# wengflow/robust-e-nerf

Measured on AMD Instinct MI355X. Metric: train_rays_per_sec, higher is better.
Workload: dtype f32; 1 GPU; BASELINE configs[1]: synthetic ficus-like event stream, 65536 events/step/GPU = 2 renders x 65536 rays x 128 samples, arch ngp, fp32, l_diff (2 renders), fwd+bwd+Adam; sampler=uniform; sampler=uniform, samples_per_ray=128, parallelism=dp1, front_prefetched=False, mlp_precision=highest, device_counts=False, device_count_overflows=0, fwd_chunks=8, dist_world_size=1

## Files before the change

robust_e_nerf_amd/csrc/ren_hashgrid_binned.hip:

```cpp
#include <cstdlib>
#include "ren_hashgrid_common.h"

namespace {

constexpr int BIN_SHIFT = 13;
constexpr int BIN_ENTRIES = 1 << BIN_SHIFT;
constexpr int MAX_BINS_PER_LEVEL = 64;
constexpr int MAX_BINS = REN_MAX_LEVELS * MAX_BINS_PER_LEVEL;
#ifndef REN_SC_THREADS
#define REN_SC_THREADS 512
#endif
#ifndef REN_SC_WAVES
#define REN_SC_WAVES 6
#endif
#ifndef REN_SC_WAVES_PAIR
#define REN_SC_WAVES_PAIR 8
#endif
constexpr int SC_THREADS = REN_SC_THREADS;
constexpr int SC_ENTRIES = SC_THREADS * 8;
constexpr int CNT_THREADS = 1024, CNT_SAMPLES = 1024;
constexpr int64_t PART_ENTRIES_MIN = 1 << 16, PART_ENTRIES_MAX = 1 << 23;
constexpr int N_SUB = 8;
__device__ __forceinline__ int xcd_id() {
    unsigned x;
    asm volatile("s_getreg_b32 %0, hwreg(HW_REG_XCC_ID)" : "=s"(x));
    return (int)(x & (N_SUB - 1));
}
inline int64_t part_entries_for(int64_t n, int64_t hashed_cap) {
    int64_t p = hashed_cap;
    if (p == 0) {
        p = PART_ENTRIES_MIN;
        while (p < (1 << 21) && p * 1024 < n * 128) p <<= 1;
    }
    return p < PART_ENTRIES_MIN ? PART_ENTRIES_MIN : (p > PART_ENTRIES_MAX ? PART_ENTRIES_MAX : p);
}
constexpr int LMAX_SLOTS = 8, LMAX_STRIDE = 32;
constexpr int LMAX_WORDS = REN_MAX_LEVELS * LMAX_SLOTS * LMAX_STRIDE;

struct BinTab {
    int bin_base[REN_MAX_LEVELS + 1];
    uint32_t cap[REN_MAX_LEVELS];
    uint32_t pair[REN_MAX_LEVELS];
    uint32_t skip[REN_MAX_LEVELS];
    int sub_by_xcd;
    int cnt_stride;
    int halve;
};

struct Part {
    uint32_t gbin, single;
    uint64_t begin, end;
};

struct Workspace {
    uint32_t *counts, *level_max, *cursors, *n_parts;
    uint32_t *bin_cap;
    uint64_t *bin_start;
    Part *parts;
    char *pool;
};
constexpr int PAIR_BIN_SHIFT = 26;

struct TanSrc {
    const float *rays_do, *rays_dd, *dfeatd;
};

__device__ __forceinline__ void lds_barrier() { asm volatile("s_waitcnt lgkmcnt(0)\n\ts_barrier" ::: "memory"); }

struct SampleArgs {
    int layout;
    const float *dfeat, *x_unit;
    ren_scene_dev sc;
    const float *rays_o, *rays_d;
    const int32_t *ray_indices;
    const float *t_starts, *t_ends;
    int64_t n;
    TanSrc tan;
    const int64_t *n_dev;
};

template <bool TAN>
__device__ __forceinline__ void unit_pos(const SampleArgs &a, int64_t i, float *u, float *ud) {
    ud[0] = 0.f; ud[1] = 0.f; ud[2] = 0.f;
    if (TAN) {
        float x[3], xd[3];
        sample_pos_jvp(a.rays_o, a.rays_d, a.tan.rays_do, a.tan.rays_dd, a.ray_indices, a.t_starts, a.t_ends, i, x, xd);
        contract_jvp(a.sc, x, xd, u, ud);
    } else if (a.x_unit) {
        u[0] = a.x_unit[3 * i]; u[1] = a.x_unit[3 * i + 1]; u[2] = a.x_unit[3 * i + 2];
    } else {
        float x, y, z; int ray;
        ren_sample_pos(a.rays_o, a.rays_d, a.ray_indices, a.t_starts, a.t_ends, i, x, y, z, ray);
        ren_contract(a.sc, x, y, z, u[0], u[1], u[2]);
    }
}

template <bool TAN>
__device__ __forceinline__ bool load_dfeat(const SampleArgs &a, int n_levels, int lvl, int64_t i, float &d0, float &d1,
                                           float &e0, float &e1) {
    e0 = 0.f; e1 = 0.f;
    if (TAN || a.layout == 1) {
        const int64_t b = ((i >> 5) * REN_MAX_LEVELS + lvl) * 64 + (i & 31);
        d0 = a.dfeat[b]; d1 = a.dfeat[b + 32];
        if (TAN) { e0 = a.tan.dfeatd[b]; e1 = a.tan.dfeatd[b + 32]; }
    } else {
        const float2 d = reinterpret_cast<const float2 *>(a.dfeat)[i * n_levels + lvl];
        d0 = d.x; d1 = d.y;
    }
    return d0 != 0.f || d1 != 0.f || e0 != 0.f || e1 != 0.f;
}


constexpr int RUN_LANES = 16;

template <int OFF>
__device__ __forceinline__ float dpp_shr(float v) {
    return __int_as_float(__builtin_amdgcn_update_dpp(0, __float_as_int(v), 0x110 | OFF, 0xf, 0xf, true));
}
template <int OFF>
__device__ __forceinline__ int dpp_shr_i(int v) { return __builtin_amdgcn_update_dpp(0, v, 0x110 | OFF, 0xf, 0xf, true); }

__device__ __forceinline__ bool run_tail(bool dense, bool have, uint32_t key, int lane, bool &head) {
    if (!dense) { head = true; return have; }
    const uint32_t k = have ? key : 0x80000000u | (uint32_t)lane;
    const uint32_t kp = __shfl_up(k, 1, 64), kn = __shfl_down(k, 1, 64);
    const int sub = lane & (RUN_LANES - 1);
    head = !(sub > 0 && have && kp == k);
    return have && (sub == RUN_LANES - 1 || kn != k);
}

template <int OFF>
__device__ __forceinline__ void run_merge_step(int &f, float (&v0)[8], float (&v1)[8]) {
    const float take = f ? 0.f : 1.f;
#pragma unroll
    for (int c = 0; c < 8; ++c) {
        v0[c] = fmaf(dpp_shr<OFF>(v0[c]), take, v0[c]);
        v1[c] = fmaf(dpp_shr<OFF>(v1[c]), take, v1[c]);
    }
    f |= dpp_shr_i<OFF>(f);
}

__device__ __forceinline__ void run_merge(bool head, int lane, float (&v0)[8], float (&v1)[8]) {
    int f = head ? 1 : 0;
    run_merge_step<1>(f, v0, v1);
    run_merge_step<2>(f, v0, v1);
    run_merge_step<4>(f, v0, v1);
    run_merge_step<8>(f, v0, v1);
}

__device__ __forceinline__ uint32_t bin_rank(bool dense, bool emit, uint32_t bin, int lane, uint32_t *hist) {
    if (!dense) return emit ? atomicAdd(&hist[bin], 1u) : 0u;
    uint32_t rank = 0;
    uint64_t todo = __ballot(emit);
    while (todo) {
        const int leader = __ffsll((unsigned long long)todo) - 1;
        const uint32_t b = __shfl(bin, leader, 64);
        const uint64_t m = __ballot(emit && bin == b);
        uint32_t base = 0;
        if (lane == leader) base = atomicAdd(&hist[b], (uint32_t)__popcll(m));
        base = __shfl(base, leader, 64);
        if (emit && bin == b) rank = base + (uint32_t)__popcll(m & ((1ull << lane) - 1ull));
        todo &= ~m;
    }
    return rank;
}

__device__ __forceinline__ void bin_rank8_dense(bool emit, const uint32_t (&bin)[8], int lane, uint32_t *hist, uint32_t (&rank)[8]) {
    const uint64_t m = __ballot(emit);
#pragma unroll
    for (int c = 0; c < 8; ++c) rank[c] = 0;
    if (!m) return;
    const int leader = __ffsll((unsigned long long)m) - 1;
    uint32_t lb[8];
    bool mixed = false;
#pragma unroll
    for (int c = 0; c < 8; ++c) {
        lb[c] = __shfl(bin[c], leader, 64);
        mixed |= emit && bin[c] != lb[c];
    }
    if (__ballot(mixed)) {
#pragma unroll
        for (int c = 0; c < 8; ++c) rank[c] = bin_rank(true, emit, bin[c], lane, hist);
        return;
    }
    const uint32_t cnt = (uint32_t)__popcll(m), pre = (uint32_t)__popcll(m & ((1ull << lane) - 1ull));
    uint32_t base[8] = {0, 0, 0, 0, 0, 0, 0, 0};
    if (lane == leader) {
#pragma unroll
        for (int c = 0; c < 8; ++c) base[c] = atomicAdd(&hist[lb[c]], cnt);
    }
#pragma unroll
    for (int c = 0; c < 8; ++c) rank[c] = __shfl(base[c], leader, 64) + pre;
}

template <bool TAN>
__global__ __launch_bounds__(CNT_THREADS) void bin_count_kernel(GridDev g, BinTab bt, SampleArgs a,
                                                                uint32_t *__restrict__ counts) {
    __shared__ uint32_t hist[MAX_BINS];
    for (int t = threadIdx.x; t < MAX_BINS; t += CNT_THREADS) hist[t] = 0;
    __syncthreads();
    const int lane = threadIdx.x & 63;
#pragma unroll 1
    for (int k = 0; k < CNT_SAMPLES / CNT_THREADS; ++k) {
        const int64_t i = (int64_t)blockIdx.x * bt.cnt_stride * CNT_SAMPLES + k * CNT_THREADS + threadIdx.x;
        const bool inb = i < ren_eff_n(a.n, a.n_dev);
        float u[3] = {0.f, 0.f, 0.f}, ud[3];
        if (inb) unit_pos<TAN>(a, i, u, ud);
#pragma unroll 1
        for (int lvl = 0; lvl < g.n_levels; ++lvl) {
            if (bt.cap[lvl] || bt.skip[lvl]) continue;
            float d0, d1, e0, e1;
            const bool have = inb && (a.dfeat == nullptr || load_dfeat<TAN>(a, g.n_levels, lvl, i, d0, d1, e0, e1));
            const LevelPos p = level_pos(u[0], u[1], u[2], g.scale[lvl]);
            const uint32_t res = g.res[lvl], size = g.size[lvl];
            const bool hashed = g.hashed[lvl] != 0;
            bool head;
            uint32_t idx[8];
            corner_indices8(p.c[0], p.c[1], p.c[2], res, size, hashed, idx);
            const bool emit = run_tail(!hashed, have, idx[0], lane, head);
#pragma unroll
            for (int c = 0; c < 8; ++c) (void)bin_rank(!hashed, emit, idx[c] >> BIN_SHIFT, lane, hist + lvl * MAX_BINS_PER_LEVEL);
        }
    }
    __syncthreads();
    for (int t = threadIdx.x; t < MAX_BINS; t += CNT_THREADS) {
        const int lvl = t / MAX_BINS_PER_LEVEL, bin = t % MAX_BINS_PER_LEVEL;
        if (lvl < g.n_levels && bin < bt.bin_base[lvl + 1] - bt.bin_base[lvl] && hist[t])
            atomicAdd(&counts[bt.bin_base[lvl] + bin], hist[t]);
    }
}

__global__ __launch_bounds__(MAX_BINS) void bin_offsets_kernel(int n_bins, BinTab bt, uint64_t capacity_slots,
                                                               const uint32_t *__restrict__ counts,
                                                               uint32_t *__restrict__ cursors,
                                                               uint32_t *__restrict__ bin_cap,
                                                               uint64_t *__restrict__ bin_start) {
    __shared__ uint64_t s_cnt[MAX_BINS];
    const int t = threadIdx.x;
    uint64_t c = 0, slots = 0;
    bool pair = false;
    if (t < n_bins) {
        int lvl = 0;
        while (lvl + 1 < REN_MAX_LEVELS && t >= bt.bin_base[lvl + 1]) ++lvl;
        pair = bt.pair[lvl] != 0;
        c = bt.skip[lvl] ? 0 : bt.cap[lvl] ? bt.cap[lvl] : counts[t];
        if (!bt.skip[lvl] && !bt.cap[lvl] && bt.cnt_stride > 1) c = c * bt.cnt_stride + c * bt.cnt_stride / 4 + 4096;
        if (bt.halve) c = c / 2;
        c &= ~(uint64_t)7;
        if (pair) c = (c / N_SUB) & ~(uint64_t)7;
        slots = pair ? c * N_SUB : (c * 10 + 15) / 16;
        for (int x = 0; x < N_SUB; ++x) cursors[t * N_SUB + x] = 0;
    }
    s_cnt[t] = slots;
    __syncthreads();
    for (int off = 1; off < MAX_BINS; off <<= 1) {
        const uint64_t a = t >= off ? s_cnt[t - off] : 0;
        __syncthreads();
        s_cnt[t] += a;
        __syncthreads();
    }
    if (t < n_bins) {
        const uint64_t start = s_cnt[t] - slots;
        uint64_t room = start < capacity_slots ? capacity_slots - start : 0;
        if (room > slots) room = slots;
        if (room < slots) c = (pair ? room / N_SUB : room * 16 / 10) & ~(uint64_t)7;
        bin_start[t] = start < capacity_slots ? start : capacity_slots;
        bin_cap[t] = (uint32_t)c;
    }
    if (t == n_bins - 1) bin_start[n_bins] = s_cnt[t] < capacity_slots ? s_cnt[t] : capacity_slots;
}

__global__ __launch_bounds__(MAX_BINS) void bin_partition_kernel(int n_bins, uint64_t PART_ENTRIES, BinTab bt,
                                                                 const uint32_t *__restrict__ cursors,
                                                                 const uint32_t *__restrict__ bin_cap,
                                                                 Part *__restrict__ parts, uint32_t *__restrict__ n_parts) {
    __shared__ uint32_t s_np[MAX_BINS];
    const int t = threadIdx.x;
    uint64_t c = 0;
    bool pair = false;
    if (t < n_bins) {
        int lvl = 0;
        while (lvl + 1 < REN_MAX_LEVELS && t >= bt.bin_base[lvl + 1]) ++lvl;
        pair = bt.pair[lvl] != 0;
        for (int x = 0; x < (pair ? N_SUB : 1); ++x) c += cursors[t * N_SUB + x] < bin_cap[t] ? cursors[t * N_SUB + x] : bin_cap[t];
    }
    const uint32_t np = pair ? (c ? 1u : 0u) : (uint32_t)((c + PART_ENTRIES - 1) / PART_ENTRIES);
    s_np[t] = np;
    __syncthreads();
    for (int off = 1; off < MAX_BINS; off <<= 1) {
        const uint32_t b = t >= off ? s_np[t - off] : 0;
        __syncthreads();
        s_np[t] += b;
        __syncthreads();
    }
    if (t == n_bins - 1) n_parts[0] = s_np[t];
    const uint32_t pbase = s_np[t] - np;
    for (uint32_t k = 0; k < np; ++k) {
        Part p;
        p.gbin = t; p.single = np == 1;
        p.begin = (uint64_t)k * PART_ENTRIES;
        p.end = k + 1 == np ? c : p.begin + PART_ENTRIES;
        parts[pbase + k] = p;
    }
}

__device__ __forceinline__ void table_atomic(float *grad_table, uint32_t offset, uint32_t idx, float a, float b) {
    float *gt = grad_table + 2 * ((size_t)offset + idx);
    atomicAdd(gt, a);
    atomicAdd(gt + 1, b);
}

template <bool TAN, int KIND>
__global__ __launch_bounds__(SC_THREADS, KIND == 1 ? REN_SC_WAVES_PAIR : REN_SC_WAVES) void bin_scatter_kernel(
    GridDev g, BinTab bt, SampleArgs a, Workspace ws, float *__restrict__ grad_table) {
    __shared__ uint32_t hist[MAX_BINS_PER_LEVEL], loc[MAX_BINS_PER_LEVEL + 1], fit[MAX_BINS_PER_LEVEL];
    __shared__ char *gp0[MAX_BINS_PER_LEVEL], *gp1[MAX_BINS_PER_LEVEL];
    __shared__ __attribute__((aligned(16))) unsigned char stage[KIND == 1 ? SC_THREADS * 4 * 16 : SC_ENTRIES * 12];
    __shared__ float wave_max[SC_THREADS / 64];
    __shared__ int any_overflow;
    uint32_t *st_key = reinterpret_cast<uint32_t *>(stage);
    float2 *st_v = reinterpret_cast<float2 *>(stage + SC_ENTRIES * 4);
    float4 *st_p = reinterpret_cast<float4 *>(stage);
    const int64_t chunk = blockIdx.x;
    const int tid = threadIdx.x, lane = tid & 63;
    const int64_t i = chunk * SC_THREADS + tid;
    const bool inb = i < ren_eff_n(a.n, a.n_dev);
    float u[3] = {0.f, 0.f, 0.f}, ud[3] = {0.f, 0.f, 0.f};
    if (inb) unit_pos<TAN>(a, i, u, ud);
    constexpr bool pairs = KIND == 1;
    const int sub = !pairs ? 0 : bt.sub_by_xcd ? xcd_id() : (int)((chunk >> 3) & (N_SUB - 1));
#pragma unroll 1
    for (int lvl = 0; lvl < g.n_levels; ++lvl) {
        if (bt.skip[lvl]) continue;
        if (KIND == 1 && !bt.pair[lvl]) continue;
        if (KIND == 2 && bt.pair[lvl]) continue;
        if (tid < MAX_BINS_PER_LEVEL) hist[tid] = 0;
        if (tid == 0) any_overflow = 0;
        lds_barrier();
        const uint32_t res = g.res[lvl], size = g.size[lvl];
        const bool hashed = g.hashed[lvl] != 0;
        const float scale = g.scale[lvl];
        float d0 = 0.f, d1 = 0.f, e0 = 0.f, e1 = 0.f;
        const bool valid = inb && load_dfeat<TAN>(a, g.n_levels, lvl, i, d0, d1, e0, e1);
        const LevelPos p = level_pos(u[0], u[1], u[2], scale);
        const float wx1 = p.w[0], wy1 = p.w[1], wz1 = p.w[2], wx0 = 1.f - wx1, wy0 = 1.f - wy1, wz0 = 1.f - wz1;
        if (!valid) { d0 = 0.f; d1 = 0.f; e0 = 0.f; e1 = 0.f; }
        uint32_t key[8];
        float v0[8], v1[8];
        bool have;
        float vmax = 0.f;
        uint32_t idx[8];
        corner_indices8(p.c[0], p.c[1], p.c[2], res, size, hashed, idx);
        if (pairs) {
            const bool same = ((idx[0] ^ idx[1]) >> BIN_SHIFT) == 0;
#pragma unroll
            for (int j = 0; j < 4; ++j) {
                const float wyz = ((j & 1) ? wy1 : wy0) * ((j & 2) ? wz1 : wz0);
                v0[j] = wyz * d0; v1[j] = wyz * d1;
            }
            if (valid && !same) {
#pragma unroll
                for (int j = 0; j < 4; ++j) {
                    table_atomic(grad_table, g.offset[lvl], idx[2 * j], wx0 * v0[j], wx0 * v1[j]);
                    table_atomic(grad_table, g.offset[lvl], idx[2 * j + 1], wx1 * v0[j], wx1 * v1[j]);
                }
            }
            have = valid && same;
#pragma unroll
            for (int j = 0; j < 4; ++j) {
                const uint32_t bin = idx[2 * j] >> BIN_SHIFT;
                key[4 + j] = have ? atomicAdd(&hist[bin], 1u) : 0u;
                key[j] = (idx[2 * j] & (BIN_ENTRIES - 1)) | ((idx[2 * j + 1] & (BIN_ENTRIES - 1)) << BIN_SHIFT) |
                         (bin << PAIR_BIN_SHIFT);
            }
            if (valid) vmax = fmaxf(fabsf(d0), fabsf(d1));
        } else {
            const float wxy[4] = {wx0 * wy0, wx1 * wy0, wx0 * wy1, wx1 * wy1};
#pragma unroll
            for (int c = 0; c < 8; ++c) {
                const float wz = (c & 4) ? wz1 : wz0;
                const float w = wxy[c & 3] * wz;
                v0[c] = w * d0; v1[c] = w * d1;
                if (TAN) {
                    const float wx = (c & 1) ? wx1 : wx0, wy = (c & 2) ? wy1 : wy0;
                    const float bx = (c & 1) ? ud[0] : -ud[0], by = (c & 2) ? ud[1] : -ud[1], bz = (c & 4) ? ud[2] : -ud[2];
                    const float wdc = scale * (bx * wy * wz + wx * by * wz + wxy[c & 3] * bz);
                    v0[c] += wdc * e0; v1[c] += wdc * e1;
                }
            }
            bool head;
            have = run_tail(!hashed, valid, idx[0], lane, head);
            if (!hashed) run_merge(head, lane, v0, v1);
            if (TAN) {
                if (have) {
#pragma unroll
                    for (int c = 0; c < 8; ++c) vmax = fmaxf(vmax, fmaxf(fabsf(v0[c]), fabsf(v1[c])));
                }
            } else if (valid) {
                vmax = fmaxf(fabsf(d0), fabsf(d1)) * (hashed ? 1.f : (float)RUN_LANES);
            }
            if (!hashed) {
                uint32_t bins[8], rk[8];
#pragma unroll
                for (int c = 0; c < 8; ++c) bins[c] = idx[c] >> BIN_SHIFT;
                bin_rank8_dense(have, bins, lane, hist, rk);
#pragma unroll
                for (int c = 0; c < 8; ++c) key[c] = (rk[c] << 19) | idx[c];
            } else {
#pragma unroll
                for (int c = 0; c < 8; ++c) {
                    const uint32_t rank = bin_rank(false, have, idx[c] >> BIN_SHIFT, lane, hist);
                    key[c] = (rank << 19) | idx[c];
                }
            }
        }
#pragma unroll
        for (int off = 32; off > 0; off >>= 1) vmax = fmaxf(vmax, __shfl_xor(vmax, off, 64));
        if (lane == 0) wave_max[tid >> 6] = vmax;
        lds_barrier();
        if (tid == SC_THREADS - 1) {
            float m = 0.f;
#pragma unroll
            for (int w = 0; w < SC_THREADS / 64; ++w) m = fmaxf(m, wave_max[w]);
            uint32_t *slot = ws.level_max + (lvl * LMAX_SLOTS + (int)(chunk % LMAX_SLOTS)) * LMAX_STRIDE;
            if (__float_as_uint(m) > __builtin_nontemporal_load(slot)) atomicMax(slot, __float_as_uint(m));
        }
        if (tid < MAX_BINS_PER_LEVEL) {
            const int nb = bt.bin_base[lvl + 1] - bt.bin_base[lvl];
            const uint32_t cnt = hist[tid];
            uint32_t inc = cnt;
#pragma unroll
            for (int off = 1; off < 64; off <<= 1) {
                const uint32_t t = __shfl_up(inc, off, 64);
                if (tid >= off) inc += t;
            }
            loc[tid] = inc - cnt;
            if (tid == MAX_BINS_PER_LEVEL - 1) loc[MAX_BINS_PER_LEVEL] = inc;
            uint32_t room = cnt;
            char *q0 = nullptr, *q1 = nullptr;
            if (tid < nb && cnt) {
                const int gb = bt.bin_base[lvl] + tid;
                const uint32_t at = atomicAdd(&ws.cursors[gb * N_SUB + sub], cnt);
                const uint32_t cap = ws.bin_cap[gb];
                room = at >= cap ? 0u : (cap - at < cnt ? cap - at : cnt);
                char *base = ws.pool + (ws.bin_start[gb] + (pairs ? (uint64_t)sub * cap : 0)) * 16;
                const int64_t first = (int64_t)at - (int64_t)(inc - cnt);
                if (pairs) q0 = base + first * 16;
                else { q0 = base + first * 8; q1 = base + (int64_t)cap * 8 + first * 2; }
            }
            fit[tid] = room;
            if (room < cnt) any_overflow = 1;
            gp0[tid] = q0; gp1[tid] = q1;
        }
        lds_barrier();
        if (have) {
            if (pairs) {
#pragma unroll
                for (int j = 0; j < 4; ++j)
                    st_p[loc[key[j] >> PAIR_BIN_SHIFT] + key[4 + j]] = make_float4(__uint_as_float(key[j]), v0[j], v1[j], wx1);
            } else {
#pragma unroll
                for (int c = 0; c < 8; ++c) {
                    const uint32_t ix = key[c] & 0x7FFFFu;
                    const uint32_t pos = loc[ix >> BIN_SHIFT] + (key[c] >> 19);
                    st_key[pos] = ix;
                    st_v[pos] = make_float2(v0[c], v1[c]);
                }
            }
        }
        lds_barrier();
        const uint32_t total = loc[MAX_BINS_PER_LEVEL];
        const bool ovf = any_overflow != 0;
        if (pairs) {
            for (uint32_t q = tid; q < total; q += SC_THREADS) {
                const float4 r = st_p[q];
                const uint32_t code = __float_as_uint(r.x), b = code >> PAIR_BIN_SHIFT;
                if (!ovf || q - loc[b] < fit[b]) {
                    reinterpret_cast<float4 *>(gp0[b])[q] = r;
                } else {
                    const uint32_t i0 = (b << BIN_SHIFT) | (code & (BIN_ENTRIES - 1));
                    const uint32_t i1 = (b << BIN_SHIFT) | ((code >> BIN_SHIFT) & (BIN_ENTRIES - 1));
                    table_atomic(grad_table, g.offset[lvl], i0, (1.f - r.w) * r.y, (1.f - r.w) * r.z);
                    table_atomic(grad_table, g.offset[lvl], i1, r.w * r.y, r.w * r.z);
                }
            }
            continue;
        }
        for (uint32_t q = tid; q < total; q += SC_THREADS) {
            const uint32_t ix = st_key[q], b = ix >> BIN_SHIFT;
            const float2 v = st_v[q];
            if (!ovf || q - loc[b] < fit[b]) {
                reinterpret_cast<uint16_t *>(gp1[b])[q] = (uint16_t)(ix & (BIN_ENTRIES - 1));
                reinterpret_cast<float2 *>(gp0[b])[q] = v;
            } else {
                table_atomic(grad_table, g.offset[lvl], ix, v.x, v.y);
            }
        }
    }
}

__device__ __forceinline__ long long to_fixed(float v, double scale) {
    return __double2ll_rn((double)v * scale);
}

__global__ __launch_bounds__(1024) void bin_accumulate_kernel(GridDev g, BinTab bt, Workspace ws,
                                                              float *__restrict__ grad_table) {
    extern __shared__ __attribute__((aligned(16))) unsigned long long acc[];
    if (blockIdx.x >= ws.n_parts[0]) return;
    const Part part = ws.parts[blockIdx.x];
    unsigned long long *acc0 = acc, *acc1 = acc + BIN_ENTRIES;
    for (int e = threadIdx.x; e < 2 * BIN_ENTRIES; e += 1024) acc[e] = 0ull;
    int lvl = 0;
    while (lvl + 1 < g.n_levels && (int)part.gbin >= bt.bin_base[lvl + 1]) ++lvl;
    int ex;
    uint32_t lmax = 0;
    for (int k = 0; k < LMAX_SLOTS; ++k) lmax = max(lmax, ws.level_max[(lvl * LMAX_SLOTS + k) * LMAX_STRIDE]);
    (void)frexpf(__uint_as_float(lmax), &ex);
    const double scale = ldexp(1.0, 38 - ex), inv_scale = ldexp(1.0, ex - 38);
    const char *base = ws.pool + ws.bin_start[part.gbin] * 16;
    const uint32_t first = ((uint32_t)part.gbin - bt.bin_base[lvl]) << BIN_SHIFT;
    const uint32_t lim = g.size[lvl] > first ? g.size[lvl] - first : 0;
    float2 *gt = reinterpret_cast<float2 *>(grad_table) + g.offset[lvl] + first;
    constexpr int FL = BIN_ENTRIES / 1024;
    float2 gv[FL];
#pragma unroll
    for (int u = 0; u < FL; ++u) {
        const uint32_t k = threadIdx.x + u * 1024;
        gv[u] = (part.single && k < lim) ? gt[k] : make_float2(0.f, 0.f);
    }
    __syncthreads();
    uint64_t e = part.begin + threadIdx.x;
    if (bt.pair[lvl]) {
        const float4 *rec = reinterpret_cast<const float4 *>(base);
        auto add = [&](const float4 &r) {
            const uint32_t code = __float_as_uint(r.x);
            const uint32_t i0 = code & (BIN_ENTRIES - 1), i1 = (code >> BIN_SHIFT) & (BIN_ENTRIES - 1);
            const float f0 = 1.f - r.w;
            atomicAdd(&acc0[i0], (unsigned long long)to_fixed(f0 * r.y, scale));
            atomicAdd(&acc1[i0], (unsigned long long)to_fixed(f0 * r.z, scale));
            atomicAdd(&acc0[i1], (unsigned long long)to_fixed(r.w * r.y, scale));
            atomicAdd(&acc1[i1], (unsigned long long)to_fixed(r.w * r.z, scale));
        };
        const uint32_t cap = ws.bin_cap[part.gbin];
        for (int x = 0; x < N_SUB; ++x) {
            const float4 *rx = rec + (size_t)x * cap;
            const uint32_t fill = ws.cursors[part.gbin * N_SUB + x];
            const uint64_t end = fill < cap ? fill : cap;
            uint64_t q = threadIdx.x;
            for (; q + 3 * 1024 < end; q += 4 * 1024) {
                float4 r[4];
#pragma unroll
                for (int u = 0; u < 4; ++u) r[u] = rx[q + u * 1024];
#pragma unroll
                for (int u = 0; u < 4; ++u) add(r[u]);
            }
            for (; q < end; q += 1024) add(rx[q]);
        }
    } else {
        const float2 *out_v = reinterpret_cast<const float2 *>(base);
        const uint16_t *out_idx = reinterpret_cast<const uint16_t *>(base + (size_t)ws.bin_cap[part.gbin] * 8);
        for (; e + 3 * 1024 < part.end; e += 4 * 1024) {
            uint32_t ix[4]; float2 v[4];
#pragma unroll
            for (int u = 0; u < 4; ++u) { ix[u] = out_idx[e + u * 1024]; v[u] = out_v[e + u * 1024]; }
#pragma unroll
            for (int u = 0; u < 4; ++u) {
                atomicAdd(&acc0[ix[u]], (unsigned long long)to_fixed(v[u].x, scale));
                atomicAdd(&acc1[ix[u]], (unsigned long long)to_fixed(v[u].y, scale));
            }
        }
        for (; e < part.end; e += 1024) {
            const uint32_t idx = out_idx[e];
            const float2 v = out_v[e];
            atomicAdd(&acc0[idx], (unsigned long long)to_fixed(v.x, scale));
            atomicAdd(&acc1[idx], (unsigned long long)to_fixed(v.y, scale));
        }
    }
    __syncthreads();
#pragma unroll
    for (int u = 0; u < FL; ++u) {
        const uint32_t k = threadIdx.x + u * 1024;
        if (k >= lim) continue;
        const long long qa = (long long)acc0[k], qb = (long long)acc1[k];
        if (qa == 0 && qb == 0) continue;
        const float a = (float)((double)qa * inv_scale), b = (float)((double)qb * inv_scale);
        if (part.single) {
            float2 v = gv[u];
            v.x += a; v.y += b;
            gt[k] = v;
        } else {
            atomicAdd(&gt[k].x, a);
            atomicAdd(&gt[k].y, b);
        }
    }
}

inline size_t align256(size_t v) { return (v + 255) & ~(size_t)255; }

struct Layout { size_t counts, level_max, cursors, n_parts, bin_cap, bin_start, parts, pool, total, slots; int64_t entries, max_parts; };

Layout make_layout(int64_t n) {
    Layout L;
    const size_t E = (size_t)n * 140 + (size_t)MAX_BINS * 4096 + 16 * 8 * 16 * CNT_SAMPLES;
    L.entries = (int64_t)E;
    L.slots = (E * 10 + 15) / 16 + MAX_BINS;
    L.max_parts = (int64_t)(E / PART_ENTRIES_MIN) + MAX_BINS + 1;
    size_t o = 0;
    L.counts = o; o += MAX_BINS * 4;
    L.level_max = o; o = align256(o + LMAX_WORDS * 4);
    L.cursors = o; o = align256(o + MAX_BINS * 4 * N_SUB);
    L.n_parts = o; o = align256(o + 4);
    L.bin_cap = o; o = align256(o + MAX_BINS * 4);
    L.bin_start = o; o = align256(o + (MAX_BINS + 1) * 8);
    L.parts = o; o = align256(o + (size_t)L.max_parts * sizeof(Part));
    L.pool = o; o = align256(o + L.slots * 16);
    L.total = o;
    return L;
}

}

extern "C" int64_t ren_hashgrid_bwd_binned_workspace_bytes(int64_t n) {
    if (n < 0) return -1;
    return (int64_t)make_layout(n).total;
}

static int binned_impl(const ren_grid_desc *grid, float *grad_table, const float *x_unit,
                       const ren_scene_desc *scene, const float *rays_o, const float *rays_d,
                       const int32_t *ray_indices, const float *t_starts, const float *t_ends,
                       int64_t n, int32_t layout, const float *dfeat, void *workspace,
                       void *stream, TanSrc tan, uint32_t level_mask = 0xFFFFFFFFu, int phases = 7,
                       int64_t first = 0, int64_t m = -1, const int64_t *n_dev = nullptr) {
    GridDev g;
    int rc = make_grid(grid, g);
    if (rc) return rc;
    const bool do_begin = phases & 1, do_scatter = phases & 2, do_finish = phases & 4;
    if (m < 0) m = n - first;
    if (!workspace || n < 0 || (layout != 0 && layout != 1) || first < 0 || m < 0 || first + m > n) return REN_ERR_BAD_ARG;
    if ((do_scatter && (!dfeat || !grad_table)) || (do_finish && !grad_table)) return REN_ERR_BAD_ARG;
    if (do_scatter && phases != 7 && ((first & 31) != 0 || tan.dfeatd)) return REN_ERR_BAD_ARG;
    const bool from_rays = x_unit == nullptr;
    if ((do_begin || do_scatter) && from_rays && (!scene || !rays_o || !rays_d || !ray_indices || !t_starts || !t_ends))
        return REN_ERR_BAD_ARG;
    if (layout == 1 && g.n_levels != REN_MAX_LEVELS) return REN_ERR_UNSUPPORTED;
    if (n >= ((int64_t)1 << 28)) return REN_ERR_UNSUPPORTED;
    BinTab bt;
    int nb = 0;
    for (int l = 0; l < REN_MAX_LEVELS; ++l) {
        bt.bin_base[l] = nb;
        if (l < g.n_levels) {
            if (g.size[l] > (uint32_t)(MAX_BINS_PER_LEVEL << BIN_SHIFT)) return REN_ERR_UNSUPPORTED;
            nb += (int)((g.size[l] + BIN_ENTRIES - 1) >> BIN_SHIFT);
        }
    }
    bt.bin_base[REN_MAX_LEVELS] = nb;
    for (int l = g.n_levels; l < REN_MAX_LEVELS; ++l) bt.bin_base[l] = nb;
    int64_t hashed_cap = 0;
    const bool use_pairs = !tan.dfeatd && ren_knob(REN_KNOB_HGB_NO_PAIRS) != 1;
    for (int l = 0; l < REN_MAX_LEVELS; ++l) {
        bt.cap[l] = 0;
        bt.pair[l] = 0;
        bt.skip[l] = l < g.n_levels && !((level_mask >> l) & 1u);
        if (l < g.n_levels && g.hashed[l]) {
            const int64_t bins = (g.size[l] + BIN_ENTRIES - 1) >> BIN_SHIFT;
            bt.pair[l] = use_pairs ? 1 : 0;
            const int64_t mean = ((use_pairs ? 4 : 8) * n + bins - 1) / bins;
            bt.cap[l] = use_pairs ? (uint32_t)(N_SUB * (((mean / N_SUB + mean / 400 + 1024) + 7) & ~(int64_t)7))
                                  : (uint32_t)(mean + mean / 50 + 4096);
            if ((int64_t)bt.cap[l] > hashed_cap) hashed_cap = bt.cap[l];
        }
    }
    const int64_t part_entries = part_entries_for(n, hashed_cap);
    if (n == 0) return REN_OK;
    ren_scene_dev sc = {};
    if (scene) sc = ren_make_scene(scene);
    const Layout L = make_layout(n);
    char *w = (char *)workspace;
    Workspace ws;
    ws.counts = (uint32_t *)(w + L.counts); ws.level_max = (uint32_t *)(w + L.level_max);
    ws.cursors = (uint32_t *)(w + L.cursors);
    ws.n_parts = (uint32_t *)(w + L.n_parts); ws.bin_cap = (uint32_t *)(w + L.bin_cap);
    ws.bin_start = (uint64_t *)(w + L.bin_start);
    ws.parts = (Part *)(w + L.parts); ws.pool = w + L.pool;
    hipStream_t st = (hipStream_t)stream;
    SampleArgs a;
    a.layout = layout; a.dfeat = dfeat; a.x_unit = x_unit; a.sc = sc; a.rays_o = rays_o; a.rays_d = rays_d;
    a.ray_indices = ray_indices; a.t_starts = t_starts; a.t_ends = t_ends; a.n = n; a.tan = tan;
    a.n_dev = n_dev;
    if (n_dev && phases != 7) return REN_ERR_BAD_ARG;
    bt.halve = ren_knob(REN_KNOB_HGB_HALVE_REGIONS) == 1;
    bt.sub_by_xcd = ren_knob(REN_KNOB_HGB_SUBREGION) != 0;
    const int64_t cnt_blocks = (n + CNT_SAMPLES - 1) / CNT_SAMPLES;
    bt.cnt_stride = cnt_blocks >= 4096 ? 16 : cnt_blocks >= 2048 ? 8 : cnt_blocks >= 1024 ? 4 : 1;
    bool any_pair = false, any_single = false;
    for (int l = 0; l < g.n_levels; ++l)
        if (!bt.skip[l]) { any_pair |= bt.pair[l] != 0; any_single |= bt.pair[l] == 0; }
    if (do_begin) {
        if (hipMemsetAsync(ws.counts, 0, (MAX_BINS + LMAX_WORDS) * 4, st) != hipSuccess) return REN_ERR_LAUNCH;
        const dim3 cgrd((unsigned)((cnt_blocks + bt.cnt_stride - 1) / bt.cnt_stride)), cblk(CNT_THREADS);
        SampleArgs ac = a;
        if (phases != 7) ac.dfeat = nullptr;
        if (tan.dfeatd) hipLaunchKernelGGL(bin_count_kernel<true>, cgrd, cblk, 0, st, g, bt, ac, ws.counts);
        else            hipLaunchKernelGGL(bin_count_kernel<false>, cgrd, cblk, 0, st, g, bt, ac, ws.counts);
        hipLaunchKernelGGL(bin_offsets_kernel, dim3(1), dim3(MAX_BINS), 0, st, nb, bt, (uint64_t)L.slots, ws.counts,
                           ws.cursors, ws.bin_cap, ws.bin_start);
    }
    if (!any_pair && !any_single) return REN_OK;
    if (do_scatter && m > 0) {
        SampleArgs as = a;
        as.n = m;
        if (first) {
            if (as.x_unit) as.x_unit += 3 * first;
            if (as.ray_indices) { as.ray_indices += first; as.t_starts += first; as.t_ends += first; }
            as.dfeat += layout == 1 ? (first >> 5) * (int64_t)(REN_MAX_LEVELS * 64) : first * (int64_t)g.n_levels * 2;
        }
        const dim3 sgrd((unsigned)((m + SC_THREADS - 1) / SC_THREADS)), sblk(SC_THREADS);
        if (tan.dfeatd) hipLaunchKernelGGL((bin_scatter_kernel<true, 0>), sgrd, sblk, 0, st, g, bt, as, ws, grad_table);
        else {
            if (any_pair)   hipLaunchKernelGGL((bin_scatter_kernel<false, 1>), sgrd, sblk, 0, st, g, bt, as, ws, grad_table);
            if (any_single) hipLaunchKernelGGL((bin_scatter_kernel<false, 2>), sgrd, sblk, 0, st, g, bt, as, ws, grad_table);
        }
    }
    if (do_finish) {
        hipLaunchKernelGGL(bin_partition_kernel, dim3(1), dim3(MAX_BINS), 0, st, nb, (uint64_t)part_entries, bt, ws.cursors, ws.bin_cap, ws.parts,
                           ws.n_parts);
        const size_t acc_lds = 2 * BIN_ENTRIES * sizeof(unsigned long long);
        (void)hipFuncSetAttribute((const void *)bin_accumulate_kernel, hipFuncAttributeMaxDynamicSharedMemorySize, (int)acc_lds);
        const int64_t acc_grid = (int64_t)(L.entries / part_entries) + nb + 1;
        hipLaunchKernelGGL(bin_accumulate_kernel, dim3((unsigned)acc_grid), dim3(1024), acc_lds, st, g, bt, ws, grad_table);
    }
    REN_CHECK_LAUNCH();
}

extern "C" int ren_hashgrid_bwd_binned(const ren_grid_desc *grid, float *grad_table, const float *x_unit,
                                       const ren_scene_desc *scene, const float *rays_o, const float *rays_d,
                                       const int32_t *ray_indices, const float *t_starts, const float *t_ends,
                                       int64_t n, int32_t layout, const float *dfeat, void *workspace,
                                       const int64_t *n_dev, void *stream) {
    return binned_impl(grid, grad_table, x_unit, scene, rays_o, rays_d, ray_indices, t_starts, t_ends, n, layout,
                       dfeat, workspace, stream, TanSrc{nullptr, nullptr, nullptr}, 0xFFFFFFFFu, 7, 0, -1, n_dev);
}

extern "C" int ren_hashgrid_bwd_binned_jvp(const ren_grid_desc *grid, float *grad_table,
                                           const ren_scene_desc *scene, const float *rays_o, const float *rays_d,
                                           const float *rays_do, const float *rays_dd, const int32_t *ray_indices,
                                           const float *t_starts, const float *t_ends, int64_t n,
                                           const float *dfeat, const float *dfeatd, void *workspace, void *stream) {
    if (!rays_do || !rays_dd || !dfeatd) return REN_ERR_BAD_ARG;
    return binned_impl(grid, grad_table, nullptr, scene, rays_o, rays_d, ray_indices, t_starts, t_ends, n, 1, dfeat,
                       workspace, stream, TanSrc{rays_do, rays_dd, dfeatd});
}

extern "C" int ren_hashgrid_bwd_binned_levels(const ren_grid_desc *grid, float *grad_table, const float *x_unit,
                                              const ren_scene_desc *scene, const float *rays_o, const float *rays_d,
                                              const int32_t *ray_indices, const float *t_starts, const float *t_ends,
                                              int64_t n, int32_t layout, const float *dfeat, const float *rays_do,
                                              const float *rays_dd, const float *dfeatd, uint32_t level_mask,
                                              void *workspace, const int64_t *n_dev, void *stream) {
    if ((rays_do || rays_dd || dfeatd) && (!rays_do || !rays_dd || !dfeatd || layout != 1 || x_unit)) return REN_ERR_BAD_ARG;
    return binned_impl(grid, grad_table, x_unit, scene, rays_o, rays_d, ray_indices, t_starts, t_ends, n, layout, dfeat,
                       workspace, stream, TanSrc{rays_do, rays_dd, dfeatd}, level_mask, 7, 0, -1, n_dev);
}

extern "C" int ren_hashgrid_bwd_binned_begin(const ren_grid_desc *grid, const float *x_unit, const ren_scene_desc *scene,
                                             const float *rays_o, const float *rays_d, const int32_t *ray_indices,
                                             const float *t_starts, const float *t_ends, int64_t n, int32_t layout,
                                             void *workspace, void *stream) {
    return binned_impl(grid, nullptr, x_unit, scene, rays_o, rays_d, ray_indices, t_starts, t_ends, n, layout, nullptr,
                       workspace, stream, TanSrc{nullptr, nullptr, nullptr}, 0xFFFFFFFFu, 1);
}

extern "C" int ren_hashgrid_bwd_binned_scatter(const ren_grid_desc *grid, float *grad_table, const float *x_unit,
                                               const ren_scene_desc *scene, const float *rays_o, const float *rays_d,
                                               const int32_t *ray_indices, const float *t_starts, const float *t_ends,
                                               int64_t n, int32_t layout, const float *dfeat, int64_t first, int64_t m,
                                               void *workspace, void *stream) {
    return binned_impl(grid, grad_table, x_unit, scene, rays_o, rays_d, ray_indices, t_starts, t_ends, n, layout, dfeat,
                       workspace, stream, TanSrc{nullptr, nullptr, nullptr}, 0xFFFFFFFFu, 2, first, m);
}

extern "C" int ren_hashgrid_bwd_binned_finish(const ren_grid_desc *grid, float *grad_table, int64_t n, int32_t layout,
                                              void *workspace, void *stream) {
    return binned_impl(grid, grad_table, nullptr, nullptr, nullptr, nullptr, nullptr, nullptr, nullptr, n, layout, nullptr,
                       workspace, stream, TanSrc{nullptr, nullptr, nullptr}, 0xFFFFFFFFu, 4);
}
```

Baseline: 5.963 million rays/s.

## Replace atomic pair-bin cursors with per-workgroup slabs and segment tables

Pair-mode hash-grid backward scatter no longer claims space in per-bin pools with global atomic cursors split into XCD sub-regions. Each scatter workgroup now writes its locally sorted records into its own slab and records a per-bin offset/count word in a segment table. The accumulate kernel walks every chunk's segment for its bin, with prefetching and lane grouping. Partial chunks are handled through a coverage bitmask. The intent is to drop the global atomics and the overflow fallback path, at the cost of the accumulate kernel scanning every chunk for every bin.

```diff
diff --git a/robust_e_nerf_amd/csrc/ren_hashgrid_binned.hip b/robust_e_nerf_amd/csrc/ren_hashgrid_binned.hip
--- a/robust_e_nerf_amd/csrc/ren_hashgrid_binned.hip
+++ b/robust_e_nerf_amd/csrc/ren_hashgrid_binned.hip
@@ -20,12 +20,10 @@
 constexpr int SC_ENTRIES = SC_THREADS * 8;
 constexpr int CNT_THREADS = 1024, CNT_SAMPLES = 1024;
 constexpr int64_t PART_ENTRIES_MIN = 1 << 16, PART_ENTRIES_MAX = 1 << 23;
-constexpr int N_SUB = 8;
-__device__ __forceinline__ int xcd_id() {
-    unsigned x;
-    asm volatile("s_getreg_b32 %0, hwreg(HW_REG_XCC_ID)" : "=s"(x));
-    return (int)(x & (N_SUB - 1));
-}
+constexpr int SLAB_RECORDS = SC_THREADS * 4;
+constexpr int SLAB_SHIFT = 9;
+static_assert(SC_THREADS == 1 << SLAB_SHIFT, "a slab is one scatter workgroup's samples");
+constexpr uint32_t PIECES = 0xFFFFFFFFu;
 inline int64_t part_entries_for(int64_t n, int64_t hashed_cap) {
     int64_t p = hashed_cap;
     if (p == 0) {
@@ -42,7 +40,6 @@
     uint32_t cap[REN_MAX_LEVELS];
     uint32_t pair[REN_MAX_LEVELS];
     uint32_t skip[REN_MAX_LEVELS];
-    int sub_by_xcd;
     int cnt_stride;
     int halve;
 };
@@ -58,6 +55,10 @@
     uint64_t *bin_start;
     Part *parts;
     char *pool;
+    float4 *slabs;
+    uint32_t *seg;
+    uint32_t *cover;
+    int64_t n_chunks;
 };
 constexpr int PAIR_BIN_SHIFT = 26;
 
@@ -75,6 +76,7 @@
     const int32_t *ray_indices;
     const float *t_starts, *t_ends;
     int64_t n;
+    int64_t lo, hi, chunk0;
     TanSrc tan;
     const int64_t *n_dev;
 };
@@ -208,7 +210,7 @@
         if (inb) unit_pos<TAN>(a, i, u, ud);
 #pragma unroll 1
         for (int lvl = 0; lvl < g.n_levels; ++lvl) {
-            if (bt.cap[lvl] || bt.skip[lvl]) continue;
+            if (bt.cap[lvl] || bt.pair[lvl] || bt.skip[lvl]) continue;
             float d0, d1, e0, e1;
             const bool have = inb && (a.dfeat == nullptr || load_dfeat<TAN>(a, g.n_levels, lvl, i, d0, d1, e0, e1));
             const LevelPos p = level_pos(u[0], u[1], u[2], g.scale[lvl]);
@@ -238,18 +240,16 @@
     __shared__ uint64_t s_cnt[MAX_BINS];
     const int t = threadIdx.x;
     uint64_t c = 0, slots = 0;
-    bool pair = false;
     if (t < n_bins) {
         int lvl = 0;
         while (lvl + 1 < REN_MAX_LEVELS && t >= bt.bin_base[lvl + 1]) ++lvl;
-        pair = bt.pair[lvl] != 0;
-        c = bt.skip[lvl] ? 0 : bt.cap[lvl] ? bt.cap[lvl] : counts[t];
-        if (!bt.skip[lvl] && !bt.cap[lvl] && bt.cnt_stride > 1) c = c * bt.cnt_stride + c * bt.cnt_stride / 4 + 4096;
+        const bool none = bt.skip[lvl] || bt.pair[lvl];
+        c = none ? 0 : bt.cap[lvl] ? bt.cap[lvl] : counts[t];
+        if (!none && !bt.cap[lvl] && bt.cnt_stride > 1) c = c * bt.cnt_stride + c * bt.cnt_stride / 4 + 4096;
         if (bt.halve) c = c / 2;
-        c &= ~(uint64_t)7;
-        if (pair) c = (c / N_SUB) & ~(uint64_t)7;
-        slots = pair ? c * N_SUB : (c * 10 + 15) / 16;
-        for (int x = 0; x < N_SUB; ++x) cursors[t * N_SUB + x] = 0;
+        c = (c + 7) & ~(uint64_t)7;
+        slots = (c * 10 + 15) / 16;
+        cursors[t] = 0;
     }
     s_cnt[t] = slots;
     __syncthreads();
@@ -263,7 +263,7 @@
         const uint64_t start = s_cnt[t] - slots;
         uint64_t room = start < capacity_slots ? capacity_slots - start : 0;
         if (room > slots) room = slots;
-        if (room < slots) c = (pair ? room / N_SUB : room * 16 / 10) & ~(uint64_t)7;
+        if (room < slots) c = (room * 16 / 10) & ~(uint64_t)7;
         bin_start[t] = start < capacity_slots ? start : capacity_slots;
         bin_cap[t] = (uint32_t)c;
     }
@@ -281,10 +281,10 @@
     if (t < n_bins) {
         int lvl = 0;
         while (lvl + 1 < REN_MAX_LEVELS && t >= bt.bin_base[lvl + 1]) ++lvl;
-        pair = bt.pair[lvl] != 0;
-        for (int x = 0; x < (pair ? N_SUB : 1); ++x) c += cursors[t * N_SUB + x] < bin_cap[t] ? cursors[t * N_SUB + x] : bin_cap[t];
-    }
-    const uint32_t np = pair ? (c ? 1u : 0u) : (uint32_t)((c + PART_ENTRIES - 1) / PART_ENTRIES);
+        pair = bt.pair[lvl] != 0 && !bt.skip[lvl];
+        c = cursors[t] < bin_cap[t] ? cursors[t] : bin_cap[t];
+    }
+    const uint32_t np = pair ? 1u : (uint32_t)((c + PART_ENTRIES - 1) / PART_ENTRIES);
     s_np[t] = np;
     __syncthreads();
     for (int off = 1; off < MAX_BINS; off <<= 1) {
@@ -321,21 +321,28 @@
     uint32_t *st_key = reinterpret_cast<uint32_t *>(stage);
     float2 *st_v = reinterpret_cast<float2 *>(stage + SC_ENTRIES * 4);
     float4 *st_p = reinterpret_cast<float4 *>(stage);
-    const int64_t chunk = blockIdx.x;
+    const int64_t chunk = a.chunk0 + blockIdx.x;
     const int tid = threadIdx.x, lane = tid & 63;
     const int64_t i = chunk * SC_THREADS + tid;
-    const bool inb = i < ren_eff_n(a.n, a.n_dev);
+    const int64_t n_eff = ren_eff_n(a.n, a.n_dev);
+    const int64_t c_lo = chunk * SC_THREADS, c_hi = c_lo + SC_THREADS, c_end = n_eff < c_hi ? n_eff : c_hi;
+    const int64_t wg_lo = a.lo > c_lo ? a.lo : c_lo, wg_hi = a.hi < c_end ? a.hi : c_end;
+    if (wg_lo >= wg_hi) return;
+    const bool inb = i >= wg_lo && i < wg_hi;
     float u[3] = {0.f, 0.f, 0.f}, ud[3] = {0.f, 0.f, 0.f};
     if (inb) unit_pos<TAN>(a, i, u, ud);
     constexpr bool pairs = KIND == 1;
-    const int sub = !pairs ? 0 : bt.sub_by_xcd ? xcd_id() : (int)((chunk >> 3) & (N_SUB - 1));
+    const bool piece = pairs && (wg_lo != c_lo || wg_hi != c_end);
+    const uint32_t piece_at = (uint32_t)(wg_lo - c_lo) * 4;
+    const uint32_t piece_len = (((uint32_t)(wg_hi - wg_lo) + 31u) & ~31u) * 4;
+    if (piece && tid == 0) atomicOr(&ws.cover[chunk], ((1u << (piece_len >> 7)) - 1u) << (piece_at >> 7));
 #pragma unroll 1
     for (int lvl = 0; lvl < g.n_levels; ++lvl) {
         if (bt.skip[lvl]) continue;
         if (KIND == 1 && !bt.pair[lvl]) continue;
         if (KIND == 2 && bt.pair[lvl]) continue;
         if (tid < MAX_BINS_PER_LEVEL) hist[tid] = 0;
-        if (tid == 0) any_overflow = 0;
+        if (!pairs && tid == 0) any_overflow = 0;
         lds_barrier();
         const uint32_t res = g.res[lvl], size = g.size[lvl];
         const bool hashed = g.hashed[lvl] != 0;
@@ -436,21 +443,26 @@
             }
             loc[tid] = inc - cnt;
             if (tid == MAX_BINS_PER_LEVEL - 1) loc[MAX_BINS_PER_LEVEL] = inc;
-            uint32_t room = cnt;
-            char *q0 = nullptr, *q1 = nullptr;
-            if (tid < nb && cnt) {
-                const int gb = bt.bin_base[lvl] + tid;
-                const uint32_t at = atomicAdd(&ws.cursors[gb * N_SUB + sub], cnt);
-                const uint32_t cap = ws.bin_cap[gb];
-                room = at >= cap ? 0u : (cap - at < cnt ? cap - at : cnt);
-                char *base = ws.pool + (ws.bin_start[gb] + (pairs ? (uint64_t)sub * cap : 0)) * 16;
-                const int64_t first = (int64_t)at - (int64_t)(inc - cnt);
-                if (pairs) q0 = base + first * 16;
-                else { q0 = base + first * 8; q1 = base + (int64_t)cap * 8 + first * 2; }
-            }
-            fit[tid] = room;
-            if (room < cnt) any_overflow = 1;
-            gp0[tid] = q0; gp1[tid] = q1;
+            if (pairs) {
+                if (tid < nb)
+                    ws.seg[((int64_t)(bt.pair[lvl] - 1) * MAX_BINS_PER_LEVEL + tid) * ws.n_chunks + chunk] =
+                        piece ? PIECES : (inc - cnt) | (cnt << 16);
+            } else {
+                uint32_t room = cnt;
+                char *q0 = nullptr, *q1 = nullptr;
+                if (tid < nb && cnt) {
+                    const int gb = bt.bin_base[lvl] + tid;
+                    const uint32_t at = atomicAdd(&ws.cursors[gb], cnt);
+                    const uint32_t cap = ws.bin_cap[gb];
+                    room = at >= cap ? 0u : (cap - at < cnt ? cap - at : cnt);
+                    char *base = ws.pool + ws.bin_start[gb] * 16;
+                    const int64_t first = (int64_t)at - (int64_t)(inc - cnt);
+                    q0 = base + first * 8; q1 = base + (int64_t)cap * 8 + first * 2;
+                }
+                fit[tid] = room;
+                if (room < cnt) any_overflow = 1;
+                gp0[tid] = q0; gp1[tid] = q1;
+            }
         }
         lds_barrier();
         if (have) {
@@ -470,22 +482,17 @@
         }
         lds_barrier();
         const uint32_t total = loc[MAX_BINS_PER_LEVEL];
+        if (pairs) {
+            float4 *slab = ws.slabs + ((int64_t)(bt.pair[lvl] - 1) * ws.n_chunks + chunk) * SLAB_RECORDS;
+            if (!piece) {
+                for (uint32_t q = tid; q < total; q += SC_THREADS) slab[q] = st_p[q];
+            } else {
+                for (uint32_t q = tid; q < piece_len; q += SC_THREADS)
+                    slab[piece_at + q] = q < total ? st_p[q] : make_float4(0.f, 0.f, 0.f, 0.f);
+            }
+            continue;
+        }
         const bool ovf = any_overflow != 0;
-        if (pairs) {
-            for (uint32_t q = tid; q < total; q += SC_THREADS) {
-                const float4 r = st_p[q];
-                const uint32_t code = __float_as_uint(r.x), b = code >> PAIR_BIN_SHIFT;
-                if (!ovf || q - loc[b] < fit[b]) {
-                    reinterpret_cast<float4 *>(gp0[b])[q] = r;
-                } else {
-                    const uint32_t i0 = (b << BIN_SHIFT) | (code & (BIN_ENTRIES - 1));
-                    const uint32_t i1 = (b << BIN_SHIFT) | ((code >> BIN_SHIFT) & (BIN_ENTRIES - 1));
-                    table_atomic(grad_table, g.offset[lvl], i0, (1.f - r.w) * r.y, (1.f - r.w) * r.z);
-                    table_atomic(grad_table, g.offset[lvl], i1, r.w * r.y, r.w * r.z);
-                }
-            }
-            continue;
-        }
         for (uint32_t q = tid; q < total; q += SC_THREADS) {
             const uint32_t ix = st_key[q], b = ix >> BIN_SHIFT;
             const float2 v = st_v[q];
@@ -503,7 +510,8 @@
     return __double2ll_rn((double)v * scale);
 }
 
-__global__ __launch_bounds__(1024) void bin_accumulate_kernel(GridDev g, BinTab bt, Workspace ws,
+__global__ __launch_bounds__(1024) void bin_accumulate_kernel(GridDev g, BinTab bt, Workspace ws, int64_t n,
+                                                              const int64_t *__restrict__ n_dev,
                                                               float *__restrict__ grad_table) {
     extern __shared__ __attribute__((aligned(16))) unsigned long long acc[];
     if (blockIdx.x >= ws.n_parts[0]) return;
@@ -531,7 +539,6 @@
     __syncthreads();
     uint64_t e = part.begin + threadIdx.x;
     if (bt.pair[lvl]) {
-        const float4 *rec = reinterpret_cast<const float4 *>(base);
         auto add = [&](const float4 &r) {
             const uint32_t code = __float_as_uint(r.x);
             const uint32_t i0 = code & (BIN_ENTRIES - 1), i1 = (code >> BIN_SHIFT) & (BIN_ENTRIES - 1);
@@ -541,20 +548,49 @@
             atomicAdd(&acc0[i1], (unsigned long long)to_fixed(r.w * r.y, scale));
             atomicAdd(&acc1[i1], (unsigned long long)to_fixed(r.w * r.z, scale));
         };
-        const uint32_t cap = ws.bin_cap[part.gbin];
-        for (int x = 0; x < N_SUB; ++x) {
-            const float4 *rx = rec + (size_t)x * cap;
-            const uint32_t fill = ws.cursors[part.gbin * N_SUB + x];
-            const uint64_t end = fill < cap ? fill : cap;
-            uint64_t q = threadIdx.x;
-            for (; q + 3 * 1024 < end; q += 4 * 1024) {
-                float4 r[4];
-#pragma unroll
-                for (int u = 0; u < 4; ++u) r[u] = rx[q + u * 1024];
-#pragma unroll
-                for (int u = 0; u < 4; ++u) add(r[u]);
-            }
-            for (; q < end; q += 1024) add(rx[q]);
+        const int nb = bt.bin_base[lvl + 1] - bt.bin_base[lvl];
+        const uint32_t bin = (uint32_t)part.gbin - (uint32_t)bt.bin_base[lvl];
+        const int lanes_shift = nb > 32 ? 3 : nb > 16 ? 4 : nb > 8 ? 5 : 6;
+        const int L = 1 << lanes_shift, G = 64 >> lanes_shift;
+        const int lane = threadIdx.x & 63, wave = threadIdx.x >> 6, sub = lane & (L - 1);
+        const int64_t chunks = (ren_eff_n(n, n_dev) + SC_THREADS - 1) >> SLAB_SHIFT;
+        const int64_t h = (int64_t)bt.pair[lvl] - 1;
+        const uint32_t *seg = ws.seg + (h * MAX_BINS_PER_LEVEL + bin) * ws.n_chunks;
+        const float4 *slabs = ws.slabs + h * ws.n_chunks * SLAB_RECORDS;
+        const int64_t step = (int64_t)(1024 / 64) * G;
+        int64_t c = (int64_t)wave * G + (lane >> lanes_shift);
+        constexpr int NF = 8;
+        auto fetch = [&](uint32_t w, int64_t ch, float4 (&r)[NF]) {
+            const uint32_t cnt = w == PIECES ? 0u : w >> 16;
+            const float4 *sl = slabs + ch * SLAB_RECORDS + (w & 0xFFFFu);
+#pragma unroll
+            for (int u = 0; u < NF; ++u) r[u] = sub + u * L < cnt ? sl[sub + u * L] : make_float4(0.f, 0.f, 0.f, 0.f);
+        };
+        uint32_t w = c < chunks ? seg[c] : 0u, w1 = c + step < chunks ? seg[c + step] : 0u;
+        float4 r[NF], rn[NF];
+        fetch(w, c, r);
+        for (int64_t c0 = (int64_t)wave * G; c0 < chunks; c0 += step, c += step) {
+            const uint32_t w2 = c + 2 * step < chunks ? seg[c + 2 * step] : 0u;
+            fetch(w1, c + step, rn);
+            const uint32_t cnt = w == PIECES ? 0u : w >> 16;
+#pragma unroll
+            for (int u = 0; u < NF; ++u)
+                if (sub + u * L < cnt) add(r[u]);
+            if (w == PIECES) {
+                const uint32_t cov = ws.cover[c];
+                const float4 *sl = slabs + c * SLAB_RECORDS;
+                for (uint32_t q = sub; q < SLAB_RECORDS; q += L) {
+                    if (!((cov >> (q >> 7)) & 1u)) continue;
+                    const float4 t = sl[q];
+                    if ((__float_as_uint(t.x) >> PAIR_BIN_SHIFT) == bin && (t.y != 0.f || t.z != 0.f)) add(t);
+                }
+            } else if (cnt > (uint32_t)(NF * L)) {
+                const float4 *sl = slabs + c * SLAB_RECORDS + (w & 0xFFFFu);
+                for (uint32_t q = sub + NF * L; q < cnt; q += L) add(sl[q]);
+            }
+#pragma unroll
+            for (int u = 0; u < NF; ++u) r[u] = rn[u];
+            w = w1; w1 = w2;
         }
     } else {
         const float2 *out_v = reinterpret_cast<const float2 *>(base);
@@ -608,7 +644,7 @@
     size_t o = 0;
     L.counts = o; o += MAX_BINS * 4;
     L.level_max = o; o = align256(o + LMAX_WORDS * 4);
-    L.cursors = o; o = align256(o + MAX_BINS * 4 * N_SUB);
+    L.cursors = o; o = align256(o + MAX_BINS * 4);
     L.n_parts = o; o = align256(o + 4);
     L.bin_cap = o; o = align256(o + MAX_BINS * 4);
     L.bin_start = o; o = align256(o + (MAX_BINS + 1) * 8);
@@ -616,6 +652,17 @@
     L.pool = o; o = align256(o + L.slots * 16);
     L.total = o;
     return L;
+}
+
+struct PairArea { int64_t chunks; size_t seg_slot, cover_slot, slots; };
+
+PairArea pair_area(int64_t n, int pair_levels) {
+    PairArea A;
+    A.chunks = (n + SC_THREADS - 1) >> SLAB_SHIFT;
+    A.seg_slot = (size_t)pair_levels * A.chunks * SLAB_RECORDS;
+    A.cover_slot = A.seg_slot + (size_t)pair_levels * A.chunks * (MAX_BINS_PER_LEVEL * 4 / 16);
+    A.slots = pair_levels ? A.cover_slot + (size_t)(A.chunks + 3) / 4 : 0;
+    return A;
 }
 
 }
@@ -656,6 +703,7 @@
     bt.bin_base[REN_MAX_LEVELS] = nb;
     for (int l = g.n_levels; l < REN_MAX_LEVELS; ++l) bt.bin_base[l] = nb;
     int64_t hashed_cap = 0;
+    int pair_levels = 0;
     const bool use_pairs = !tan.dfeatd && ren_knob(REN_KNOB_HGB_NO_PAIRS) != 1;
     for (int l = 0; l < REN_MAX_LEVELS; ++l) {
         bt.cap[l] = 0;
@@ -663,11 +711,11 @@
         bt.skip[l] = l < g.n_levels && !((level_mask >> l) & 1u);
         if (l < g.n_levels && g.hashed[l]) {
             const int64_t bins = (g.size[l] + BIN_ENTRIES - 1) >> BIN_SHIFT;
-            bt.pair[l] = use_pairs ? 1 : 0;
             const int64_t mean = ((use_pairs ? 4 : 8) * n + bins - 1) / bins;
-            bt.cap[l] = use_pairs ? (uint32_t)(N_SUB * (((mean / N_SUB + mean / 400 + 1024) + 7) & ~(int64_t)7))
-                                  : (uint32_t)(mean + mean / 50 + 4096);
-            if ((int64_t)bt.cap[l] > hashed_cap) hashed_cap = bt.cap[l];
+            const int64_t c = use_pairs ? 8 * (((mean / 8 + mean / 400 + 1024) + 7) & ~(int64_t)7) : mean + mean / 50 + 4096;
+            if (use_pairs) bt.pair[l] = (uint32_t)++pair_levels;
+            else bt.cap[l] = (uint32_t)c;
+            if (c > hashed_cap) hashed_cap = c;
         }
     }
     const int64_t part_entries = part_entries_for(n, hashed_cap);
@@ -681,15 +729,22 @@
     ws.cursors = (uint32_t *)(w + L.cursors);
     ws.n_parts = (uint32_t *)(w + L.n_parts); ws.bin_cap = (uint32_t *)(w + L.bin_cap);
     ws.bin_start = (uint64_t *)(w + L.bin_start);
-    ws.parts = (Part *)(w + L.parts); ws.pool = w + L.pool;
+    ws.parts = (Part *)(w + L.parts);
+    const PairArea A = pair_area(n, pair_levels);
+    if (A.slots > L.slots) return REN_ERR_UNSUPPORTED;
+    ws.slabs = (float4 *)(w + L.pool);
+    ws.seg = (uint32_t *)(w + L.pool + A.seg_slot * 16);
+    ws.cover = (uint32_t *)(w + L.pool + A.cover_slot * 16);
+    ws.n_chunks = A.chunks;
+    ws.pool = w + L.pool + A.slots * 16;
     hipStream_t st = (hipStream_t)stream;
     SampleArgs a;
     a.layout = layout; a.dfeat = dfeat; a.x_unit = x_unit; a.sc = sc; a.rays_o = rays_o; a.rays_d = rays_d;
     a.ray_indices = ray_indices; a.t_starts = t_starts; a.t_ends = t_ends; a.n = n; a.tan = tan;
+    a.lo = 0; a.hi = n; a.chunk0 = 0;
     a.n_dev = n_dev;
     if (n_dev && phases != 7) return REN_ERR_BAD_ARG;
     bt.halve = ren_knob(REN_KNOB_HGB_HALVE_REGIONS) == 1;
-    bt.sub_by_xcd = ren_knob(REN_KNOB_HGB_SUBREGION) != 0;
     const int64_t cnt_blocks = (n + CNT_SAMPLES - 1) / CNT_SAMPLES;
     bt.cnt_stride = cnt_blocks >= 4096 ? 16 : cnt_blocks >= 2048 ? 8 : cnt_blocks >= 1024 ? 4 : 1;
     bool any_pair = false, any_single = false;
@@ -697,24 +752,20 @@
         if (!bt.skip[l]) { any_pair |= bt.pair[l] != 0; any_single |= bt.pair[l] == 0; }
     if (do_begin) {
         if (hipMemsetAsync(ws.counts, 0, (MAX_BINS + LMAX_WORDS) * 4, st) != hipSuccess) return REN_ERR_LAUNCH;
+        if (phases != 7 && pair_levels && hipMemsetAsync(ws.cover, 0, (size_t)A.chunks * 4, st) != hipSuccess) return REN_ERR_LAUNCH;
         const dim3 cgrd((unsigned)((cnt_blocks + bt.cnt_stride - 1) / bt.cnt_stride)), cblk(CNT_THREADS);
         SampleArgs ac = a;
         if (phases != 7) ac.dfeat = nullptr;
         if (tan.dfeatd) hipLaunchKernelGGL(bin_count_kernel<true>, cgrd, cblk, 0, st, g, bt, ac, ws.counts);
         else            hipLaunchKernelGGL(bin_count_kernel<false>, cgrd, cblk, 0, st, g, bt, ac, ws.counts);
-        hipLaunchKernelGGL(bin_offsets_kernel, dim3(1), dim3(MAX_BINS), 0, st, nb, bt, (uint64_t)L.slots, ws.counts,
+        hipLaunchKernelGGL(bin_offsets_kernel, dim3(1), dim3(MAX_BINS), 0, st, nb, bt, (uint64_t)(L.slots - A.slots), ws.counts,
                            ws.cursors, ws.bin_cap, ws.bin_start);
     }
     if (!any_pair && !any_single) return REN_OK;
     if (do_scatter && m > 0) {
         SampleArgs as = a;
-        as.n = m;
-        if (first) {
-            if (as.x_unit) as.x_unit += 3 * first;
-            if (as.ray_indices) { as.ray_indices += first; as.t_starts += first; as.t_ends += first; }
-            as.dfeat += layout == 1 ? (first >> 5) * (int64_t)(REN_MAX_LEVELS * 64) : first * (int64_t)g.n_levels * 2;
-        }
-        const dim3 sgrd((unsigned)((m + SC_THREADS - 1) / SC_THREADS)), sblk(SC_THREADS);
+        as.lo = first; as.hi = first + m; as.chunk0 = first >> SLAB_SHIFT;
+        const dim3 sgrd((unsigned)(((first + m - 1) >> SLAB_SHIFT) - as.chunk0 + 1)), sblk(SC_THREADS);
         if (tan.dfeatd) hipLaunchKernelGGL((bin_scatter_kernel<true, 0>), sgrd, sblk, 0, st, g, bt, as, ws, grad_table);
         else {
             if (any_pair)   hipLaunchKernelGGL((bin_scatter_kernel<false, 1>), sgrd, sblk, 0, st, g, bt, as, ws, grad_table);
@@ -727,7 +778,7 @@
         const size_t acc_lds = 2 * BIN_ENTRIES * sizeof(unsigned long long);
         (void)hipFuncSetAttribute((const void *)bin_accumulate_kernel, hipFuncAttributeMaxDynamicSharedMemorySize, (int)acc_lds);
         const int64_t acc_grid = (int64_t)(L.entries / part_entries) + nb + 1;
-        hipLaunchKernelGGL(bin_accumulate_kernel, dim3((unsigned)acc_grid), dim3(1024), acc_lds, st, g, bt, ws, grad_table);
+        hipLaunchKernelGGL(bin_accumulate_kernel, dim3((unsigned)acc_grid), dim3(1024), acc_lds, st, g, bt, ws, n, n_dev, grad_table);
     }
     REN_CHECK_LAUNCH();
 }
```

Measured after the change: 6.005 million rays/s (median of 6 runs). No clear change (+0.7%).
